# ErlerPhilipp/points2surf

Measured on NVIDIA H100. Metric: SDF queries/sec at grid_res=256, higher is better.
Workload: dtype f16 operands / f32 accumulate (wgmma); hi/lo split f16 (fp32-level) for FC tails and guard-band recompute

## Files before the change

points2surf_b200/csrc/net_tc.cu:

```cuda
#include "model.cuh"
#include "tc_ptx.cuh"

namespace p2s {

using namespace ptx;

namespace {

constexpr int kTile = 64;
constexpr int kWG = 2;
constexpr int kThreads = 128 * kWG;
template <bool PRECISE>
struct Cfg {
    static constexpr int kChunks = PRECISE ? 2 : 4;
    static constexpr int kSplit = 8 / kChunks;
    static constexpr uint32_t kChunkBytes = PRECISE ? 65536u : 32768u;
    static constexpr uint32_t kW3Bytes = kChunks * kChunkBytes;
    static constexpr uint32_t kMidScale = PRECISE ? 2u : 1u;
    static constexpr uint32_t kMidBytes = (8192u + 8192u + 16384u) * kMidScale;
    static constexpr uint32_t kPerqBytes = PRECISE ? 16384u : 8192u;
    static constexpr uint32_t kRedBytes = 4u * kChunks * 128u * 4u;
    static constexpr uint32_t kOffMid = kW3Bytes;
    static constexpr uint32_t kWgWq = kPerqBytes;
    static constexpr uint32_t kWgBytes = kWgWq + 192 * 4;
    static constexpr uint32_t kOffWg = kOffMid + kMidBytes;
    static constexpr uint32_t kOffBias = kOffWg + kWG * kWgBytes;
    static constexpr uint32_t kSlotBytes = PRECISE ? 0u : 8u * 128u * 16u;
    static constexpr uint32_t kOffSlot = kOffBias + 320 * 4;
    static constexpr uint32_t kOffXBar = kOffSlot + kWG * kSlotBytes;
    static constexpr uint32_t kSmemBytes = kOffXBar + (PRECISE ? 0u : kWG * 16u);
};
static_assert(Cfg<false>::kSmemBytes <= 232448 && Cfg<true>::kSmemBytes <= 232448, "shared memory budget");
static_assert(Cfg<false>::kRedBytes <= Cfg<false>::kPerqBytes && Cfg<true>::kRedBytes <= Cfg<true>::kPerqBytes, "reduction scratch");

struct Seg {
    const float* ptr;
    int n;
    int tiles;
    int center;
};

struct PassParams {
    Seg seg[2];
    const float* query;
    const float* R;
    int tiles_per_query;
    int B;
    const float* W0;
    const float* b0;
    int num_mid;
    int mid_N[3];
    const uint8_t* mid_img[3];
    const float* mid_bias[3];
    int perq_layer;
    const uint8_t* perq_img;
    const uint8_t* w3_img;
    float* out;
};

__device__ __forceinline__ uint32_t pack_relu(float a, float b) {
    uint32_t r;
    asm("cvt.rn.relu.satfinite.f16x2.f32 %0, %1, %2;" : "=r"(r) : "f"(b), "f"(a));
    return r;
}
__device__ __forceinline__ void pack_relu_split(float a, float b, uint32_t& hi, uint32_t& lo) {
    hi = pack_relu(a, b);
    const float2 hf = __half22float2(*reinterpret_cast<const __half2*>(&hi));
    lo = pack_half2(fmaxf(a, 0.f) - hf.x, fmaxf(b, 0.f) - hf.y);
}
template <bool PRECISE>
__device__ __forceinline__ void pack_act(float a, float b, uint32_t& hi, uint32_t& lo) {
    if (PRECISE) pack_relu_split(a, b, hi, lo);
    else hi = pack_relu(a, b);
}

template <bool PRECISE, int R>
__device__ __forceinline__ void mid_mma(float (&d)[R], const uint32_t (&a)[4], const uint32_t (&al)[4], uint64_t w, uint64_t w_lo, uint32_t acc) {
    if (R == 32) {
        auto& d32 = reinterpret_cast<float (&)[32]>(d);
        if (PRECISE) { wgmma_rs_n64(d32, al, w, acc); wgmma_rs_n64(d32, a, w_lo, 1); wgmma_rs_n64(d32, a, w, 1); }
        else wgmma_rs_n64(d32, a, w, acc);
    } else {
        auto& d64 = reinterpret_cast<float (&)[64]>(d);
        if (PRECISE) { wgmma_rs_n128(d64, al, w, acc); wgmma_rs_n128(d64, a, w_lo, 1); wgmma_rs_n128(d64, a, w, 1); }
        else wgmma_rs_n128(d64, a, w, acc);
    }
}

template <bool PRECISE, int R, int KL>
__device__ __forceinline__ void pack_acc(const float (&d)[R], const float* bias, int q4, uint32_t (&a)[R / 8][4], uint32_t (&al)[R / 8][KL]) {
#pragma unroll
    for (int j = 0; j < R / 4; ++j) {
        const float2 bb = *reinterpret_cast<const float2*>(bias + 8 * j + 2 * q4);
        pack_act<PRECISE>(d[4 * j] + bb.x, d[4 * j + 1] + bb.y, a[j >> 1][(j & 1) * 2], al[j >> 1][PRECISE ? (j & 1) * 2 : 0]);
        pack_act<PRECISE>(d[4 * j + 2] + bb.x, d[4 * j + 3] + bb.y, a[j >> 1][(j & 1) * 2 + 1], al[j >> 1][PRECISE ? (j & 1) * 2 + 1 : 0]);
    }
}

template <int S>
__device__ __forceinline__ void max_halve(float (&m)[32], int lane) {
    const bool up = (lane & S) != 0;
#pragma unroll
    for (int i = 0; i < S; ++i) {
        const float send = up ? m[i] : m[i + S], keep = up ? m[i + S] : m[i];
        m[i] = fmaxf(keep, __shfl_xor_sync(0xffffffffu, send, S));
    }
}

template <bool PRECISE>
__global__ void __launch_bounds__(kThreads, 1) pointnet_pass_kernel(const PassParams p) {
    using C = Cfg<PRECISE>;
    constexpr int kL = PRECISE ? 4 : 1;
    extern __shared__ __align__(1024) uint8_t smem[];
    float* s_bias = reinterpret_cast<float*>(smem + C::kOffBias);
    const int tid = threadIdx.x, wg = tid >> 7, t = tid & 127, lane = tid & 31, q4 = lane & 3;
    const int r0 = (t >> 5) * 16 + (lane >> 2);
    const int part = blockIdx.x % C::kSplit;
    const int stream = blockIdx.x / C::kSplit, nstreams = gridDim.x / C::kSplit;
    const int nq = (p.B > stream) ? (p.B - stream + nstreams - 1) / nstreams : 0;
    const int tpq = p.tiles_per_query;
    uint32_t mid_off[3] = {0, 0, 0};
    {
        uint32_t o = 0;
        for (int l = 0; l < (PRECISE ? p.num_mid : 3); ++l) {
            if (!PRECISE && l >= p.num_mid) break;
            mid_off[l] = o; o += (uint32_t)p.mid_N[l] * 128u * C::kMidScale;
        }
    }

    if (nq > 0) {
        const uint4* src = reinterpret_cast<const uint4*>(p.w3_img + (size_t)part * C::kW3Bytes);
        uint4* dst = reinterpret_cast<uint4*>(smem);
        for (uint32_t i = tid; i < C::kW3Bytes / 16; i += kThreads) dst[i] = src[i];
        for (int l = 0; l < (PRECISE ? p.num_mid : 3); ++l) {
            if (!PRECISE && l >= p.num_mid) break;
            if (l == p.perq_layer) continue;
            const uint4* s = reinterpret_cast<const uint4*>(p.mid_img[l]);
            uint4* d = reinterpret_cast<uint4*>(smem + C::kOffMid + mid_off[l]);
            for (uint32_t i = tid; i < (uint32_t)p.mid_N[l] * 8u * C::kMidScale; i += kThreads) d[i] = s[i];
        }
    }
    {
        int off = 0;
        for (int l = 0; l < p.num_mid; ++l) {
            for (int i = tid; i < p.mid_N[l]; i += kThreads) s_bias[off + i] = p.mid_bias[l][i];
            off += p.mid_N[l];
        }
        for (int i = tid; i < 64; i += kThreads) s_bias[256 + i] = p.b0[i];
    }
    uint64_t* xbar = reinterpret_cast<uint64_t*>(smem + C::kOffXBar);
    if (!PRECISE && tid == 0) {
        for (int w = 0; w < kWG; ++w) {
            mbar_init(xbar + 2 * w, 1);
            mbar_arrive_expect_tx(xbar + 2 * w, C::kSlotBytes);
            mbar_init(xbar + 2 * w + 1, 128);
        }
        fence_mbar_init();
    }
    fence_proxy_async_smem();
    __syncthreads();
    if (!PRECISE) cluster_sync();

    uint8_t* wsm = smem + C::kOffWg + wg * C::kWgBytes;
    uint8_t* perq = wsm;
    float* red = reinterpret_cast<float*>(perq);
    float* wq = reinterpret_cast<float*>(wsm + C::kWgWq);
    const float* s_b0 = s_bias + 256;
    const uint32_t bar_id = 1 + (uint32_t)wg;
    auto wg_sync = [&]() { asm volatile("bar.sync %0, 128;" ::"r"(bar_id) : "memory"); };
    const uint64_t dsc_w3 = make_smem_desc(smem_u32(smem), 128, 2048);
    uint64_t dsc_mid[3], dsc_mid_lo[3];
    for (int l = 0; l < 3; ++l) {
        const bool pq = l == p.perq_layer;
        dsc_mid[l] = make_smem_desc(pq ? smem_u32(perq) : smem_u32(smem + C::kOffMid) + mid_off[l], 128, 1024);
        dsc_mid_lo[l] = dsc_mid[l] + (uint64_t)((pq ? 8192u : (uint32_t)p.mid_N[l] * 128u) >> 4);
    }
    uint8_t* slot = smem + C::kOffSlot + wg * C::kSlotBytes;
    uint64_t* full = xbar + 2 * wg;
    uint64_t* empty = xbar + 2 * wg + 1;
    const uint32_t peer = (uint32_t)part ^ 1u;
    uint32_t nsend = 0, nrecv = 0;

    for (int qi = wg; qi < nq; qi += kWG) {
        const size_t q = (size_t)stream + (size_t)qi * nstreams;
        wg_sync();
        if (t < 64) {
            const float w0 = p.W0[t * 3 + 0], w1 = p.W0[t * 3 + 1], w2 = p.W0[t * 3 + 2];
            float r[9] = {1.f, 0.f, 0.f, 0.f, 1.f, 0.f, 0.f, 0.f, 1.f};
            if (p.R) {
#pragma unroll
                for (int i = 0; i < 9; ++i) r[i] = p.R[q * 9 + i];
            }
            wq[0 * 64 + t] = w0 * r[0] + w1 * r[3] + w2 * r[6];
            wq[1 * 64 + t] = w0 * r[1] + w1 * r[4] + w2 * r[7];
            wq[2 * 64 + t] = w0 * r[2] + w1 * r[5] + w2 * r[8];
        }
        if (p.perq_layer >= 0) {
            const uint4* s = reinterpret_cast<const uint4*>(p.perq_img + q * C::kPerqBytes);
            uint4* d = reinterpret_cast<uint4*>(perq);
            for (uint32_t i = t; i < C::kPerqBytes / 16; i += 128) d[i] = s[i];
            fence_proxy_async_smem();
        }
        wg_sync();
        float vmax[4 * C::kChunks];
#pragma unroll
        for (int i = 0; i < 4 * C::kChunks; ++i) vmax[i] = -INFINITY;
        const int own = PRECISE ? 0 : (part ^ wg ^ (qi >> 1)) & 1;
        for (int i = 0; i < tpq; ++i) {
            const int tq = PRECISE ? i : (i & ~1) + own;
            const bool mine = PRECISE || (!(i & 1) && tq < tpq);
            uint32_t a2[8][4], a2l[8][kL];
            if (mine) {
                const int sgi = tq < p.seg[0].tiles ? 0 : 1;
                const Seg& sg = p.seg[sgi];
                float cx = 0.f, cy = 0.f, cz = 0.f;
                if (sg.center) { cx = p.query[q * 3 + 0]; cy = p.query[q * 3 + 1]; cz = p.query[q * 3 + 2]; }
                float px[2], py[2], pz[2];
#pragma unroll
                for (int h = 0; h < 2; ++h) {
                    int local = (tq - (sgi ? p.seg[0].tiles : 0)) * kTile + r0 + 8 * h;
                    if (local >= sg.n) local = 0;
                    const float* src = sg.ptr + (q * sg.n + local) * 3;
                    px[h] = src[0] - cx; py[h] = src[1] - cy; pz[h] = src[2] - cz;
                }
                uint32_t a[4][4], al[4][kL];
#pragma unroll
                for (int kk = 0; kk < 4; ++kk) {
#pragma unroll
                    for (int hc = 0; hc < 2; ++hc) {
                        const int ch = kk * 16 + hc * 8 + 2 * q4;
                        const float2 wx = *reinterpret_cast<const float2*>(wq + 0 * 64 + ch);
                        const float2 wy = *reinterpret_cast<const float2*>(wq + 1 * 64 + ch);
                        const float2 wz = *reinterpret_cast<const float2*>(wq + 2 * 64 + ch);
                        const float2 bb = *reinterpret_cast<const float2*>(s_b0 + ch);
#pragma unroll
                        for (int h = 0; h < 2; ++h) {
                            const float v0 = fmaf(wx.x, px[h], fmaf(wy.x, py[h], fmaf(wz.x, pz[h], bb.x)));
                            const float v1 = fmaf(wx.y, px[h], fmaf(wy.y, py[h], fmaf(wz.y, pz[h], bb.y)));
                            pack_act<PRECISE>(v0, v1, a[kk][hc * 2 + h], al[kk][PRECISE ? hc * 2 + h : 0]);
                        }
                    }
                }
                const float* bl = s_bias;
#pragma unroll
                for (int l = 0; l < 2; ++l) {
                    if (l >= p.num_mid - 1) break;
                    float d[32];
#pragma unroll
                    for (int i = 0; i < 32; ++i) d[i] = 0.f;
                    wgmma_fence();
#pragma unroll
                    for (int ks = 0; ks < 4; ++ks)
                        mid_mma<PRECISE>(d, a[ks], reinterpret_cast<const uint32_t (&)[4]>(al[PRECISE ? ks : 0]), dsc_mid[l] + (uint64_t)(ks * 16), dsc_mid_lo[l] + (uint64_t)(ks * 16), ks > 0);
                    wgmma_commit();
                    wgmma_wait<0>();
                    fence_regs(d);
                    pack_acc<PRECISE>(d, bl, q4, a, al);
                    bl += 64;
                }
                {
                    const uint64_t w = p.num_mid == 3 ? dsc_mid[2] : dsc_mid[0], w_lo = p.num_mid == 3 ? dsc_mid_lo[2] : dsc_mid_lo[0];
                    float d[64];
#pragma unroll
                    for (int i = 0; i < 64; ++i) d[i] = 0.f;
                    wgmma_fence();
#pragma unroll
                    for (int ks = 0; ks < 4; ++ks)
                        mid_mma<PRECISE>(d, a[ks], reinterpret_cast<const uint32_t (&)[4]>(al[PRECISE ? ks : 0]), w + (uint64_t)(ks * 16), w_lo + (uint64_t)(ks * 16), ks > 0);
                    wgmma_commit();
                    wgmma_wait<0>();
                    fence_regs(d);
                    pack_acc<PRECISE>(d, bl, q4, a2, a2l);
                }
                if (!PRECISE) {
                    if (nsend > 0) mbar_wait_cluster_bounded(empty, (nsend - 1) & 1);
                    const uint32_t dst = mapa(smem_u32(slot), peer) + 16u * (uint32_t)t, bar = mapa(smem_u32(full), peer);
#pragma unroll
                    for (int k = 0; k < 8; ++k) st_async_v4(dst + 2048u * k, a2[k], bar);
                    ++nsend;
                }
            } else {
                mbar_wait_cluster_bounded(full, nrecv & 1);
#pragma unroll
                for (int k = 0; k < 8; ++k) {
                    const uint4 v = reinterpret_cast<const uint4*>(slot)[128 * k + t];
                    a2[k][0] = v.x; a2[k][1] = v.y; a2[k][2] = v.z; a2[k][3] = v.w;
                }
                mbar_arrive_cluster(mapa(smem_u32(empty), peer));
                if (t == 0) mbar_arrive_expect_tx(full, C::kSlotBytes);
                ++nrecv;
            }
#pragma unroll(PRECISE ? 1 : C::kChunks)
            for (int c = 0; c < C::kChunks; ++c) {
                float d[64];
#pragma unroll
                for (int i = 0; i < 64; ++i) d[i] = 0.f;
                const uint64_t w = dsc_w3 + (uint64_t)((uint32_t)c * (C::kChunkBytes >> 4));
                wgmma_fence();
#pragma unroll
                for (int ks = 0; ks < 8; ++ks) {
                    const uint64_t o = w + (uint64_t)(ks * 16);
                    if (PRECISE) {
                        wgmma_rs_n128(d, a2[ks], o + (uint64_t)(32768u >> 4), ks > 0);
                        wgmma_rs_n128(d, reinterpret_cast<const uint32_t (&)[4]>(a2l[PRECISE ? ks : 0]), o, 1);
                        wgmma_rs_n128(d, a2[ks], o, 1);
                    } else {
                        wgmma_rs_n128(d, a2[ks], o, ks > 0);
                    }
                }
                wgmma_commit();
                wgmma_wait<0>();
                fence_regs(d);
                float m[32];
#pragma unroll
                for (int j = 0; j < 16; ++j) {
                    m[2 * j] = fmaxf(d[4 * j], d[4 * j + 2]);
                    m[2 * j + 1] = fmaxf(d[4 * j + 1], d[4 * j + 3]);
                }
                max_halve<16>(m, lane);
                max_halve<8>(m, lane);
                max_halve<4>(m, lane);
                float v[4];
#pragma unroll
                for (int i = 0; i < 4; ++i) v[i] = fmaxf(vmax[i], m[i]);
#pragma unroll
                for (int i = 0; i < 4 * (C::kChunks - 1); ++i) vmax[i] = vmax[i + 4];
#pragma unroll
                for (int i = 0; i < 4; ++i) vmax[4 * (C::kChunks - 1) + i] = v[i];
            }
        }
        constexpr int kC = C::kChunks * 128;
        const int warp = t >> 5;
        wg_sync();
#pragma unroll
        for (int c = 0; c < C::kChunks; ++c)
#pragma unroll
            for (int h = 0; h < 2; ++h)
                *reinterpret_cast<float2*>(red + warp * kC + c * 128 + 16 * (lane >> 2) + 8 * h + 2 * q4) = make_float2(vmax[4 * c + 2 * h], vmax[4 * c + 2 * h + 1]);
        wg_sync();
        for (int i = t; i < kC / 4; i += 128) {
            const float4* r4 = reinterpret_cast<const float4*>(red);
            float4 v = r4[i];
#pragma unroll
            for (int w = 1; w < 4; ++w) {
                const float4 u = r4[w * (kC / 4) + i];
                v = make_float4(fmaxf(v.x, u.x), fmaxf(v.y, u.y), fmaxf(v.z, u.z), fmaxf(v.w, u.w));
            }
            *reinterpret_cast<float4*>(p.out + q * 1024 + (size_t)(part * kC + 4 * i)) = v;
        }
    }
    if (!PRECISE) cluster_sync();
}

__global__ void pack_kmajor_kernel(const float* __restrict__ W, int rows, int K, int row0, uint32_t sbo, uint8_t* __restrict__ img, int lo) {
    int e = blockIdx.x * blockDim.x + threadIdx.x;
    if (e >= rows * K) return;
    int r = e / K, k = e % K;
    uint32_t off = (uint32_t)(r >> 3) * sbo + (uint32_t)(k >> 3) * 128u + (uint32_t)(r & 7) * 16u + (uint32_t)(k & 7) * 2u;
    const float w = W[(size_t)(row0 + r) * K + k];
    const __half h = __float2half_rn(w);
    *reinterpret_cast<__half*>(img + off) = lo ? __float2half_rn(w - __half2float(h)) : h;
}

__global__ void pack_perq_kernel(const float* __restrict__ W, int64_t B, uint8_t* __restrict__ img) {
    int64_t e = (int64_t)blockIdx.x * blockDim.x + threadIdx.x;
    if (e >= B * 4096) return;
    int64_t b = e >> 12;
    int r = (int)((e >> 6) & 63), k = (int)(e & 63);
    uint32_t off = (uint32_t)(r >> 3) * 1024u + (uint32_t)(k >> 3) * 128u + (uint32_t)(r & 7) * 16u + (uint32_t)(k & 7) * 2u;
    *reinterpret_cast<__half*>(img + b * 8192 + off) = __float2half_rn(W[e]);
}

__global__ void __launch_bounds__(256) fold_w1_kernel(const float* __restrict__ W1, const float* __restrict__ T, int64_t B, uint8_t* __restrict__ img) {
    __shared__ float sW[64][65];
    __shared__ __align__(16) float sT[64][68];
    const int64_t b = blockIdx.x;
    const int tid = threadIdx.x;
    for (int e = tid; e < 4096; e += 256) {
        const int r = e >> 6, c = e & 63;
        sW[r][c] = W1[e];
        sT[r][c] = T[b * 4096 + e] + (r == c ? 1.0f : 0.0f);
    }
    __syncthreads();
    const int o = tid >> 2, i0 = (tid & 3) * 16;
    float acc[16];
#pragma unroll
    for (int i = 0; i < 16; ++i) acc[i] = 0.f;
    for (int j = 0; j < 64; ++j) {
        const float w = sW[o][j];
#pragma unroll
        for (int i4 = 0; i4 < 4; ++i4) {
            const float4 t4 = *reinterpret_cast<const float4*>(&sT[j][i0 + 4 * i4]);
            acc[4 * i4 + 0] = fmaf(w, t4.x, acc[4 * i4 + 0]);
            acc[4 * i4 + 1] = fmaf(w, t4.y, acc[4 * i4 + 1]);
            acc[4 * i4 + 2] = fmaf(w, t4.z, acc[4 * i4 + 2]);
            acc[4 * i4 + 3] = fmaf(w, t4.w, acc[4 * i4 + 3]);
        }
    }
    uint8_t* dst = img + b * 8192 + (uint32_t)(o >> 3) * 1024u + (uint32_t)(o & 7) * 16u;
#pragma unroll
    for (int h = 0; h < 2; ++h) {
        uint32_t v[4];
#pragma unroll
        for (int e = 0; e < 4; ++e) v[e] = pack_half2(acc[h * 8 + 2 * e], acc[h * 8 + 2 * e + 1]);
        *reinterpret_cast<uint4*>(dst + (uint32_t)(i0 / 8 + h) * 128u) = make_uint4(v[0], v[1], v[2], v[3]);
    }
}

__global__ void fold_fc3_kernel(const float* __restrict__ W1, const float* __restrict__ Wfc3, const float* __restrict__ bfc3,
                                float* __restrict__ G, float* __restrict__ g0) {
    const int oi = blockIdx.x;
    const int o = oi >> 6, i = oi & 63;
    const int k = threadIdx.x;
    float acc = 0.f;
    for (int j = 0; j < 64; ++j) acc = fmaf(W1[o * 64 + j], Wfc3[(size_t)(j * 64 + i) * 256 + k], acc);
    G[(size_t)oi * 256 + k] = acc;
    if (k == 0) {
        float b = W1[o * 64 + i];
        for (int j = 0; j < 64; ++j) b = fmaf(W1[o * 64 + j], bfc3[j * 64 + i], b);
        g0[oi] = b;
    }
}

__global__ void transpose64_kernel(const float* __restrict__ in, float* __restrict__ out, int64_t B) {
    int64_t e = (int64_t)blockIdx.x * blockDim.x + threadIdx.x;
    if (e >= B * 4096) return;
    int64_t b = e >> 12;
    int i = (int)((e >> 6) & 63), j = (int)(e & 63);
    out[e] = in[b * 4096 + j * 64 + i];
}

__global__ void guard_flag_kernel(const float* __restrict__ logits, int od, int64_t B, float band, int32_t* __restrict__ list, int* __restrict__ count, int64_t base, int64_t cap) {
    int64_t i = (int64_t)blockIdx.x * blockDim.x + threadIdx.x;
    if (i >= B) return;
    if (fabsf(logits[i * od + od - 1]) < band) {
        int slot = atomicAdd(count, 1);
        if (slot < cap) list[slot] = (int32_t)(base + i);
    }
}
__global__ void guard_gather_kernel(const float* __restrict__ src, const int32_t* __restrict__ list, int n, int row_floats, float* __restrict__ dst) {
    int64_t e = (int64_t)blockIdx.x * blockDim.x + threadIdx.x;
    if (e >= (int64_t)n * row_floats) return;
    int i = (int)(e / row_floats), j = (int)(e % row_floats);
    dst[e] = src[(int64_t)list[i] * row_floats + j];
}
__global__ void guard_scatter_kernel(const float* __restrict__ src, const int32_t* __restrict__ list, int n, int od, float* __restrict__ logits) {
    int i = blockIdx.x * blockDim.x + threadIdx.x;
    if (i >= n) return;
    for (int j = 0; j < od; ++j) logits[(int64_t)list[i] * od + j] = src[i * od + j];
}
__global__ void guard_scatter_rows_kernel(const float* __restrict__ src, const int32_t* __restrict__ list, int n, int row_floats, float* __restrict__ dst) {
    int64_t e = (int64_t)blockIdx.x * blockDim.x + threadIdx.x;
    if (e >= (int64_t)n * row_floats) return;
    int i = (int)(e / row_floats), j = (int)(e % row_floats);
    dst[(int64_t)list[i] * row_floats + j] = src[e];
}

}

struct TcStack {
    uint8_t* w3_img = nullptr;
    uint8_t* mid_img[3] = {nullptr, nullptr, nullptr};
    uint8_t* w3_img_p = nullptr;
    uint8_t* mid_img_p[3] = {nullptr, nullptr, nullptr};
    const float* mid_bias[3] = {nullptr, nullptr, nullptr};
    int mid_N[3] = {0, 0, 0};
    int num_mid = 0;
    const float* W0 = nullptr;
    const float* b0 = nullptr;
    const float* b3 = nullptr;
};

struct TcFc {
    const Layer* L = nullptr;
    const uint8_t* img = nullptr;
};
struct TcStnFc { TcFc fc1, fc2, fc3; };

struct TcWeights {
    TcStack qstn;
    TcStack stn[2], fin[2];
    TcStnFc qstn_fc, stn_fc[2];
    TcFc head_fc1[2], head_fc2, head_fc3;
    const uint8_t* fold_img[2] = {nullptr, nullptr};
    const float* fold_bias[2] = {nullptr, nullptr};
    TcStack stn_enc, fin_enc;
    TcStnFc stn_fc_enc;
    TcFc head_fc1_enc;
    const uint8_t* fold_img_enc = nullptr;
    const float* fold_bias_enc = nullptr;
    bool fc_on_tc = true;
    std::vector<void*> allocs;
    int sm_count = 132;
    int pass_clusters = 66;
    bool prof_on = false;
    std::vector<std::pair<cudaEvent_t, cudaEvent_t>> prof_events;
    double prof_flops = 0.0;
    ~TcWeights() {
        for (void* a : allocs) cudaFree(a);
        for (auto& e : prof_events) { cudaEventDestroy(e.first); cudaEventDestroy(e.second); }
    }
};

// ... 256 lines not shown
        launch_fc_tc_img(imgA, f.fc1.img, f.fc1.L->b, imgB, 0, Bc, 512, 1024, true, st, 3, 16, 0);
        if (out_f2) launch_fc_tc_img(imgB, f.fc2.img, f.fc2.L->b, out_f2, 256, Bc, 256, 512, true, st, 0);
        else launch_fc_tc_img(imgB, f.fc2.img, f.fc2.L->b, imgC, 0, Bc, 256, 512, true, st, 3, 8, 0);
    };
    auto qstn_rot = [&](const Layer& c3, int64_t Bc) {
        { StageScope ts("net: fc tails", st);
          if (fc_tc && img_ok(t.qstn_fc)) {
              stn_tail_img(c3, t.qstn_fc, gmax, Bc, f2);
              run_fc(t.qstn_fc.fc3, f2, 256, q4, 4, Bc, false, false, st);
          } else fc_tail(c3, t.qstn_fc, fc_tc, gmax, Bc, g, f1, f2, q4, st); }
        launch_quat_to_rot(q4, R, Bc, st);
    };
    auto stn64_perq = [&](const Feat& f, const TcStnFc& fc, const uint8_t* fold_img, const float* fold_bias, int64_t Bc) {
        if (fc_tc) {
            StageScope ts("net: fc tails", st);
            if (img_ok(fc)) {
                stn_tail_img(f.stn2.c3, fc, gmax, Bc, nullptr);
                launch_fc_tc_img(imgC, fold_img, fold_bias, perq, 0, Bc, 4096, 256, false, st, precise ? 2 : 1);
            } else {
                run_fc(fc.fc1, gmax, 1024, f1, 512, Bc, true, true, st, f.stn2.c3.b, true);
                run_fc(fc.fc2, f1, 512, f2, 256, Bc, true, true, st);
                launch_fc_tc(f2, 256, fold_img, fold_bias, reinterpret_cast<float*>(perq), 0, Bc, 4096, 256, false, st, precise ? 2 : 1);
            }
        } else {
            { StageScope ts("net: fc tails", st); fc_tail(f.stn2.c3, fc, false, gmax, Bc, g, f1, f2, T, st); }
            { StageScope ts("net: fold W1*T", st); P2S_LAUNCH(fold_w1_kernel, (unsigned)Bc, 256, 0, st, f.conv1.W, T, Bc, perq); }
        }
    };

    for (int64_t b0 = 0; b0 < B; b0 += Bc_max) {
        const int64_t Bc = (B - b0 < Bc_max) ? (B - b0) : Bc_max;
        const float* pa = patch + b0 * P * 3;
        const float* su = sub + b0 * S * 3;
        const float* qu = query + b0 * 3;
        const float* Rq = nullptr;
        if (m.single_transformer) {
            const Seg sp = make_seg(pa, P, 0), ss = make_seg(su, S, 1);
            { StageScope ts("net: pass kernels", st); launch_pass(m, t.qstn, sp, ss, qu, nullptr, Bc, -1, nullptr, gmax, st, precise); }
            qstn_rot(m.enc.stn1.c3, Bc);
            { StageScope ts("net: pass kernels", st); launch_pass(m, t.stn_enc, sp, ss, qu, R, Bc, -1, nullptr, gmax, st, precise); }
            stn64_perq(m.enc, t.stn_fc_enc, t.fold_img_enc, t.fold_bias_enc, Bc);
            { StageScope ts("net: pass kernels", st); launch_pass(m, t.fin_enc, sp, ss, qu, R, Bc, 1, perq, fmax_l, st, precise); }
            const bool fuse_b3 = fc_tc && !m.debug_aux && t.head_fc1_enc.img;
            if (!fuse_b3) launch_bias_act(fmax_l, m.enc.conv3.b, Bc, 1024, false, st);
            debug_aux_copy(m, b0, Bc, R, fmax_l, nullptr, st);
            StageScope ts_head("net: fc tails", st);
            if (fuse_b3 && t.head_fc2.img && t.head_fc3.img) {
                uint8_t* imgCat = reinterpret_cast<uint8_t*>(cat);
                launch_pack_a(fmax_l, 1024, Bc, 1024, m.enc.conv3.b, false, imgA, st);
                launch_fc_tc_img(imgA, t.head_fc1_enc.img, m.fc1_enc.b, imgCat, 0, Bc, 1024, 1024, true, st, 3, 32, 0);
                launch_fc_tc_img(imgCat, t.head_fc2.img, m.fc2.b, imgC, 0, Bc, 256, 1024, true, st, 3, 8, 0);
                launch_fc_tc_img(imgC, t.head_fc3.img, m.fc3.b, h4, 128, Bc, 128, 256, true, st, 0);
            } else {
                run_fc(t.head_fc1_enc, fmax_l, 1024, cat, 1024, Bc, true, fc_tc, st, fuse_b3 ? m.enc.conv3.b : nullptr, false);
                run_fc(t.head_fc2, cat, 1024, h3, 256, Bc, true, fc_tc, st);
                run_fc(t.head_fc3, h3, 256, h4, 128, Bc, true, fc_tc, st);
            }
            const int od = m.fc4.cout;
            launch_gemm_nt(h4, 0, 128, m.fc4.W, 0, m.fc4.b, logits + b0 * od, 0, od, (int)Bc, od, 128, 1, false, st);
            continue;
        }
        if (m.shared_qstn) {
            { StageScope ts("net: pass kernels", st); launch_pass(m, t.qstn, make_seg(pa, P, 0), make_seg(su, S, 1), qu, nullptr, Bc, -1, nullptr, gmax, st, precise); }
            qstn_rot(m.point_stn.c3, Bc);
            Rq = R;
        } else if (m.global.has_qstn) {
            launch_pass(m, t.qstn, make_seg(su, S, 1), make_seg(nullptr, 0, 0), qu, nullptr, Bc, -1, nullptr, gmax, st, precise);
            qstn_rot(m.global.stn1.c3, Bc);
            Rq = R;
        }
        for (int br = 1; br >= 0; --br) {
            const Feat& f = br ? m.global : m.local;
            const Seg sg = br ? make_seg(su, S, 1) : make_seg(pa, P, 0);
            float* fmax = br ? fmax_g : fmax_l;
            { StageScope ts("net: pass kernels", st); launch_pass(m, t.stn[br], sg, make_seg(nullptr, 0, 0), qu, Rq, Bc, -1, nullptr, gmax, st, precise); }
            stn64_perq(f, t.stn_fc[br], t.fold_img[br], t.fold_bias[br], Bc);
            (void)Tt;
            { StageScope ts("net: pass kernels", st); launch_pass(m, t.fin[br], sg, make_seg(nullptr, 0, 0), qu, Rq, Bc, 1, perq, fmax, st, precise); }
        }
        const bool fuse_b3 = fc_tc && !m.debug_aux && t.head_fc1[0].img && t.head_fc1[1].img;
        if (!fuse_b3) {
            launch_bias_act(fmax_l, m.local.conv3.b, Bc, 1024, false, st);
            launch_bias_act(fmax_g, m.global.conv3.b, Bc, 1024, false, st);
        }
        debug_aux_copy(m, b0, Bc, Rq, fmax_l, fmax_g, st);
        StageScope ts_head("net: fc tails", st);
        if (fuse_b3 && t.head_fc2.img && t.head_fc3.img) {
            uint8_t* imgCat = reinterpret_cast<uint8_t*>(cat);
            launch_pack_a(fmax_l, 1024, Bc, 1024, m.local.conv3.b, false, imgA, st);
            launch_fc_tc_img(imgA, t.head_fc1[0].img, m.fc1_local.b, imgCat, 0, Bc, 512, 1024, true, st, 3, 32, 0);
            launch_pack_a(fmax_g, 1024, Bc, 1024, m.global.conv3.b, false, imgA, st);
            launch_fc_tc_img(imgA, t.head_fc1[1].img, m.fc1_global.b, imgCat, 0, Bc, 512, 1024, true, st, 3, 32, 16);
            launch_fc_tc_img(imgCat, t.head_fc2.img, m.fc2.b, imgC, 0, Bc, 256, 1024, true, st, 3, 8, 0);
            launch_fc_tc_img(imgC, t.head_fc3.img, m.fc3.b, h4, 128, Bc, 128, 256, true, st, 0);
        } else {
            run_fc(t.head_fc1[0], fmax_l, 1024, cat, 1024, Bc, true, fc_tc, st, fuse_b3 ? m.local.conv3.b : nullptr, false);
            run_fc(t.head_fc1[1], fmax_g, 1024, cat + 512, 1024, Bc, true, fc_tc, st, fuse_b3 ? m.global.conv3.b : nullptr, false);
            run_fc(t.head_fc2, cat, 1024, h3, 256, Bc, true, fc_tc, st);
            run_fc(t.head_fc3, h3, 256, h4, 128, Bc, true, fc_tc, st);
        }
        const int od = m.fc4.cout;
        launch_gemm_nt(h4, 0, 128, m.fc4.W, 0, m.fc4.b, logits + b0 * od, 0, od, (int)Bc, od, 128, 1, false, st);
    }
}

void forward_guard(Model& m, const float* patch, const float* sub, const float* query, int64_t B, float* logits, cudaStream_t st) {
    static const bool use_fp32 = env_flag("P2S_GUARD_FP32");
    if (use_fp32) forward_fp32(m, patch, sub, query, B, logits, st);
    else forward_tc_core(m, patch, sub, query, B, logits, st, true);
}

void forward_tc(Model& m, const float* patch, const float* sub, const float* query, int64_t B,
                float* logits, cudaStream_t st) {
    const int P = m.cfg.points_per_patch, S = m.cfg.sub_sample_size, od = m.fc4.cout;
    forward_tc_core(m, patch, sub, query, B, logits, st, false);

    if (m.guard_band > 0.f && m.guard_list) {
        P2S_LAUNCH(guard_flag_kernel, (unsigned)cdiv(B, 256), 256, 0, st, logits, od, B, m.guard_band, m.guard_list, m.guard_list_count, m.guard_base, m.guard_list_cap);
    } else if (m.guard_band > 0.f) {
        StageScope ts_guard("net: guard-band fp32 recompute", st);
        int32_t* list = m.ws_guard.as<int32_t>((size_t)B + 64);
        int* count = reinterpret_cast<int*>(list + B);
        P2S_CUDA(cudaMemsetAsync(count, 0, sizeof(int), st));
        P2S_LAUNCH(guard_flag_kernel, (unsigned)cdiv(B, 256), 256, 0, st, logits, od, B, m.guard_band, list, count, (int64_t)0, B);
        int n = 0;
        P2S_CUDA(cudaMemcpyAsync(&n, count, sizeof(int), cudaMemcpyDeviceToHost, st));
        P2S_CUDA(cudaStreamSynchronize(st));
        m.last_guard_count += n;
        if (n > 0) {
            const size_t rowp = (size_t)P * 3, rows = (size_t)S * 3;
            float* const aux = m.debug_aux;
            const size_t aux_floats = aux ? (size_t)n * kAuxStride : 0;
            float* gbuf = m.ws_misc.as<float>((size_t)n * (rowp + rows + 3 + od) + 64 + aux_floats);
            float* gp = gbuf; float* gs = gp + (size_t)n * rowp; float* gq = gs + (size_t)n * rows; float* gl = gq + ((size_t)n * 3 + 3) / 4 * 4;
            float* gaux = gl + ((size_t)n * od + 3) / 4 * 4;
            P2S_LAUNCH(guard_gather_kernel, (unsigned)cdiv((int64_t)n * rowp, 256), 256, 0, st, patch, list, n, (int)rowp, gp);
            P2S_LAUNCH(guard_gather_kernel, (unsigned)cdiv((int64_t)n * rows, 256), 256, 0, st, sub, list, n, (int)rows, gs);
            P2S_LAUNCH(guard_gather_kernel, (unsigned)cdiv((int64_t)n * 3, 256), 256, 0, st, query, list, n, 3, gq);
            if (aux) m.debug_aux = gaux;
            try {
                forward_guard(m, gp, gs, gq, n, gl, st);
            } catch (...) {
                m.debug_aux = aux;
                throw;
            }
            m.debug_aux = aux;
            P2S_LAUNCH(guard_scatter_kernel, (unsigned)cdiv(n, 256), 256, 0, st, gl, list, n, od, logits);
            if (aux) P2S_LAUNCH(guard_scatter_rows_kernel, (unsigned)cdiv((int64_t)n * kAuxStride, 256), 256, 0, st, gaux, list, n, (int)kAuxStride, aux);
        }
    }
}

}
```

points2surf_b200/csrc/tc_ptx.cuh:

```cuda
#pragma once
#include <cstdint>
#include <cuda_fp16.h>

namespace p2s {
namespace ptx {

__device__ __forceinline__ uint32_t smem_u32(const void* p) { return (uint32_t)__cvta_generic_to_shared(p); }

__device__ __forceinline__ void mbar_init(uint64_t* bar, uint32_t count) {
    asm volatile("mbarrier.init.shared::cta.b64 [%0], %1;" ::"r"(smem_u32(bar)), "r"(count) : "memory");
}
__device__ __forceinline__ void fence_mbar_init() { asm volatile("fence.mbarrier_init.release.cluster;" ::: "memory"); }
__device__ __forceinline__ void mbar_arrive(uint64_t* bar) {
    asm volatile("mbarrier.arrive.shared::cta.b64 _, [%0];" ::"r"(smem_u32(bar)) : "memory");
}
__device__ __forceinline__ void mbar_arrive_expect_tx(uint64_t* bar, uint32_t bytes) {
    asm volatile("mbarrier.arrive.expect_tx.shared::cta.b64 _, [%0], %1;" ::"r"(smem_u32(bar)), "r"(bytes) : "memory");
}
__device__ __forceinline__ bool mbar_try_wait(uint64_t* bar, uint32_t parity) {
    uint32_t ok;
    asm volatile(
        "{\n\t.reg .pred p;\n\t"
        "mbarrier.try_wait.parity.shared::cta.b64 p, [%1], %2;\n\t"
        "selp.u32 %0, 1, 0, p;\n\t}"
        : "=r"(ok) : "r"(smem_u32(bar)), "r"(parity) : "memory");
    return ok != 0;
}
__device__ __forceinline__ void mbar_wait_bounded(uint64_t* bar, uint32_t parity) {
    long long t0 = clock64();
    while (!mbar_try_wait(bar, parity)) {
        if (clock64() - t0 > 2000000000LL) __trap();
    }
}
__device__ __forceinline__ bool mbar_test_wait(uint64_t* bar, uint32_t parity) {
    uint32_t ok;
    asm volatile(
        "{\n\t.reg .pred p;\n\t"
        "mbarrier.test_wait.parity.shared::cta.b64 p, [%1], %2;\n\t"
        "selp.u32 %0, 1, 0, p;\n\t}"
        : "=r"(ok) : "r"(smem_u32(bar)), "r"(parity) : "memory");
    return ok != 0;
}
__device__ __forceinline__ void mbar_wait(uint64_t* bar, uint32_t parity) {
    while (!mbar_try_wait(bar, parity)) {}
}

__device__ __forceinline__ uint32_t mapa(uint32_t addr, uint32_t rank) {
    uint32_t r;
    asm("mapa.shared::cluster.u32 %0, %1, %2;" : "=r"(r) : "r"(addr), "r"(rank));
    return r;
}
__device__ __forceinline__ void cluster_sync() {
    asm volatile("barrier.cluster.arrive.release;\n\tbarrier.cluster.wait.acquire;" ::: "memory");
}
__device__ __forceinline__ void st_async_v4(uint32_t addr, const uint32_t (&v)[4], uint32_t bar_addr) {
    asm volatile("st.async.shared::cluster.mbarrier::complete_tx::bytes.v4.b32 [%0], {%1, %2, %3, %4}, [%5];"
                 ::"r"(addr), "r"(v[0]), "r"(v[1]), "r"(v[2]), "r"(v[3]), "r"(bar_addr) : "memory");
}
__device__ __forceinline__ void mbar_arrive_cluster(uint32_t bar_addr) {
    asm volatile("mbarrier.arrive.release.cluster.shared::cluster.b64 _, [%0];" ::"r"(bar_addr) : "memory");
}
__device__ __forceinline__ bool mbar_try_wait_cluster(uint64_t* bar, uint32_t parity) {
    uint32_t ok;
    asm volatile(
        "{\n\t.reg .pred p;\n\t"
        "mbarrier.try_wait.parity.acquire.cluster.shared::cta.b64 p, [%1], %2;\n\t"
        "selp.u32 %0, 1, 0, p;\n\t}"
        : "=r"(ok) : "r"(smem_u32(bar)), "r"(parity) : "memory");
    return ok != 0;
}
__device__ __forceinline__ void mbar_wait_cluster_bounded(uint64_t* bar, uint32_t parity) {
    long long t0 = clock64();
    while (!mbar_try_wait_cluster(bar, parity)) {
        if (clock64() - t0 > 2000000000LL) __trap();
    }
}

__device__ __forceinline__ bool elect_one() {
    uint32_t pred;
    asm volatile("{\n\t.reg .pred P1;\n\telect.sync _|P1, 0xffffffff;\n\tselp.u32 %0, 1, 0, P1;\n\t}" : "=r"(pred));
    return pred != 0;
}

__device__ __forceinline__ void fence_proxy_async_smem() { asm volatile("fence.proxy.async.shared::cta;" ::: "memory"); }

__device__ __forceinline__ void bulk_g2s(void* smem_dst, const void* gmem_src, uint32_t bytes, uint64_t* bar) {
    asm volatile("cp.async.bulk.shared::cluster.global.mbarrier::complete_tx::bytes [%0], [%1], %2, [%3];"
                 ::"r"(smem_u32(smem_dst)), "l"(gmem_src), "r"(bytes), "r"(smem_u32(bar)) : "memory");
}

__device__ __forceinline__ uint64_t make_smem_desc(uint32_t smem_addr, uint32_t lbo_bytes, uint32_t sbo_bytes) {
    uint64_t d = 0;
    d |= (uint64_t)((smem_addr & 0x3FFFFu) >> 4);
    d |= (uint64_t)((lbo_bytes >> 4) & 0x3FFFu) << 16;
    d |= (uint64_t)((sbo_bytes >> 4) & 0x3FFFu) << 32;
    return d;
}

__device__ __forceinline__ void wgmma_fence() { asm volatile("wgmma.fence.sync.aligned;" ::: "memory"); }
__device__ __forceinline__ void wgmma_commit() { asm volatile("wgmma.commit_group.sync.aligned;" ::: "memory"); }
template <int N>
__device__ __forceinline__ void wgmma_wait() { asm volatile("wgmma.wait_group.sync.aligned %0;" ::"n"(N) : "memory"); }
template <int R>
__device__ __forceinline__ void fence_regs(float (&d)[R]) {
#pragma unroll
    for (int i = 0; i < R; ++i) asm volatile("" : "+f"(d[i])::"memory");
}
__device__ __forceinline__ void wgmma_rs_n64(float (&d)[32], const uint32_t (&a)[4], uint64_t b_desc, uint32_t accumulate) {
    asm volatile(
        "{\n\t.reg .pred p;\n\tsetp.ne.b32 p, %37, 0;\n\t"
        "wgmma.mma_async.sync.aligned.m64n64k16.f32.f16.f16 {%0, %1, %2, %3, %4, %5, %6, %7, %8, %9, %10, %11, %12, %13, %14, %15, %16, %17, %18, %19, %20, %21, %22, %23, %24, %25, %26, %27, %28, %29, %30, %31}, {%32, %33, %34, %35}, %36, p, 1, 1, 0;\n\t}"
        : "+f"(d[0]), "+f"(d[1]), "+f"(d[2]), "+f"(d[3]), "+f"(d[4]), "+f"(d[5]), "+f"(d[6]), "+f"(d[7]), "+f"(d[8]), "+f"(d[9]), "+f"(d[10]), "+f"(d[11]), "+f"(d[12]), "+f"(d[13]), "+f"(d[14]), "+f"(d[15]), "+f"(d[16]), "+f"(d[17]), "+f"(d[18]), "+f"(d[19]), "+f"(d[20]), "+f"(d[21]), "+f"(d[22]), "+f"(d[23]), "+f"(d[24]), "+f"(d[25]), "+f"(d[26]), "+f"(d[27]), "+f"(d[28]), "+f"(d[29]), "+f"(d[30]), "+f"(d[31])
        : "r"(a[0]), "r"(a[1]), "r"(a[2]), "r"(a[3]), "l"(b_desc), "r"(accumulate) : "memory");
}
__device__ __forceinline__ void wgmma_rs_n128(float (&d)[64], const uint32_t (&a)[4], uint64_t b_desc, uint32_t accumulate) {
    asm volatile(
        "{\n\t.reg .pred p;\n\tsetp.ne.b32 p, %69, 0;\n\t"
        "wgmma.mma_async.sync.aligned.m64n128k16.f32.f16.f16 {%0, %1, %2, %3, %4, %5, %6, %7, %8, %9, %10, %11, %12, %13, %14, %15, %16, %17, %18, %19, %20, %21, %22, %23, %24, %25, %26, %27, %28, %29, %30, %31, %32, %33, %34, %35, %36, %37, %38, %39, %40, %41, %42, %43, %44, %45, %46, %47, %48, %49, %50, %51, %52, %53, %54, %55, %56, %57, %58, %59, %60, %61, %62, %63}, {%64, %65, %66, %67}, %68, p, 1, 1, 0;\n\t}"
        : "+f"(d[0]), "+f"(d[1]), "+f"(d[2]), "+f"(d[3]), "+f"(d[4]), "+f"(d[5]), "+f"(d[6]), "+f"(d[7]), "+f"(d[8]), "+f"(d[9]), "+f"(d[10]), "+f"(d[11]), "+f"(d[12]), "+f"(d[13]), "+f"(d[14]), "+f"(d[15]), "+f"(d[16]), "+f"(d[17]), "+f"(d[18]), "+f"(d[19]), "+f"(d[20]), "+f"(d[21]), "+f"(d[22]), "+f"(d[23]), "+f"(d[24]), "+f"(d[25]), "+f"(d[26]), "+f"(d[27]), "+f"(d[28]), "+f"(d[29]), "+f"(d[30]), "+f"(d[31]), "+f"(d[32]), "+f"(d[33]), "+f"(d[34]), "+f"(d[35]), "+f"(d[36]), "+f"(d[37]), "+f"(d[38]), "+f"(d[39]), "+f"(d[40]), "+f"(d[41]), "+f"(d[42]), "+f"(d[43]), "+f"(d[44]), "+f"(d[45]), "+f"(d[46]), "+f"(d[47]), "+f"(d[48]), "+f"(d[49]), "+f"(d[50]), "+f"(d[51]), "+f"(d[52]), "+f"(d[53]), "+f"(d[54]), "+f"(d[55]), "+f"(d[56]), "+f"(d[57]), "+f"(d[58]), "+f"(d[59]), "+f"(d[60]), "+f"(d[61]), "+f"(d[62]), "+f"(d[63])
        : "r"(a[0]), "r"(a[1]), "r"(a[2]), "r"(a[3]), "l"(b_desc), "r"(accumulate) : "memory");
}
__device__ __forceinline__ void wgmma_ss_n128(float (&d)[64], uint64_t a_desc, uint64_t b_desc, uint32_t accumulate) {
    asm volatile(
        "{\n\t.reg .pred p;\n\tsetp.ne.b32 p, %66, 0;\n\t"
        "wgmma.mma_async.sync.aligned.m64n128k16.f32.f16.f16 {%0, %1, %2, %3, %4, %5, %6, %7, %8, %9, %10, %11, %12, %13, %14, %15, %16, %17, %18, %19, %20, %21, %22, %23, %24, %25, %26, %27, %28, %29, %30, %31, %32, %33, %34, %35, %36, %37, %38, %39, %40, %41, %42, %43, %44, %45, %46, %47, %48, %49, %50, %51, %52, %53, %54, %55, %56, %57, %58, %59, %60, %61, %62, %63}, %64, %65, p, 1, 1, 0, 0;\n\t}"
        : "+f"(d[0]), "+f"(d[1]), "+f"(d[2]), "+f"(d[3]), "+f"(d[4]), "+f"(d[5]), "+f"(d[6]), "+f"(d[7]), "+f"(d[8]), "+f"(d[9]), "+f"(d[10]), "+f"(d[11]), "+f"(d[12]), "+f"(d[13]), "+f"(d[14]), "+f"(d[15]), "+f"(d[16]), "+f"(d[17]), "+f"(d[18]), "+f"(d[19]), "+f"(d[20]), "+f"(d[21]), "+f"(d[22]), "+f"(d[23]), "+f"(d[24]), "+f"(d[25]), "+f"(d[26]), "+f"(d[27]), "+f"(d[28]), "+f"(d[29]), "+f"(d[30]), "+f"(d[31]), "+f"(d[32]), "+f"(d[33]), "+f"(d[34]), "+f"(d[35]), "+f"(d[36]), "+f"(d[37]), "+f"(d[38]), "+f"(d[39]), "+f"(d[40]), "+f"(d[41]), "+f"(d[42]), "+f"(d[43]), "+f"(d[44]), "+f"(d[45]), "+f"(d[46]), "+f"(d[47]), "+f"(d[48]), "+f"(d[49]), "+f"(d[50]), "+f"(d[51]), "+f"(d[52]), "+f"(d[53]), "+f"(d[54]), "+f"(d[55]), "+f"(d[56]), "+f"(d[57]), "+f"(d[58]), "+f"(d[59]), "+f"(d[60]), "+f"(d[61]), "+f"(d[62]), "+f"(d[63])
        : "l"(a_desc), "l"(b_desc), "r"(accumulate) : "memory");
}

__device__ __forceinline__ uint32_t pack_half2(float lo, float hi) {
    __half2 h = __floats2half2_rn(lo, hi);
    return *reinterpret_cast<uint32_t*>(&h);
}

}
}
```

Baseline: 431,800.

## Prefetch point tiles via cp.async and double-buffer big-layer wgmma chunks

In the fast (non-precise) path, each warp prefetches the next tile's points into shared memory with cp.async, so the first layer no longer waits on global loads. The big layer's wgmma chunks are double-buffered across two accumulator sets, and the max-reduction of one chunk overlaps the next chunk's MMA. The release of the peer's empty slot moves to after the first chunk completes and is predicated on whether the tile was received. Holding two 64-float accumulator sets raises register pressure, and optional clock-based phase tracing is added behind a compile flag.

```diff
diff --git a/points2surf_b200/csrc/net_tc.cu b/points2surf_b200/csrc/net_tc.cu
--- a/points2surf_b200/csrc/net_tc.cu
+++ b/points2surf_b200/csrc/net_tc.cu
@@ -28,7 +28,9 @@
     static constexpr uint32_t kSlotBytes = PRECISE ? 0u : 8u * 128u * 16u;
     static constexpr uint32_t kOffSlot = kOffBias + 320 * 4;
     static constexpr uint32_t kOffXBar = kOffSlot + kWG * kSlotBytes;
-    static constexpr uint32_t kSmemBytes = kOffXBar + (PRECISE ? 0u : kWG * 16u);
+    static constexpr uint32_t kPtsBytes = PRECISE ? 0u : 16u * 3u * 4u;
+    static constexpr uint32_t kOffPts = kOffXBar + (PRECISE ? 0u : kWG * 16u);
+    static constexpr uint32_t kSmemBytes = kOffPts + kWG * 4u * kPtsBytes;
 };
 static_assert(Cfg<false>::kSmemBytes <= 232448 && Cfg<true>::kSmemBytes <= 232448, "shared memory budget");
 static_assert(Cfg<false>::kRedBytes <= Cfg<false>::kPerqBytes && Cfg<true>::kRedBytes <= Cfg<true>::kPerqBytes, "reduction scratch");
@@ -106,6 +108,50 @@
         m[i] = fmaxf(keep, __shfl_xor_sync(0xffffffffu, send, S));
     }
 }
+
+template <int kChunks>
+__device__ __forceinline__ void max_chunk(const float (&d)[64], float (&vmax)[4 * kChunks], int lane) {
+    float m[32];
+#pragma unroll
+    for (int j = 0; j < 16; ++j) {
+        m[2 * j] = fmaxf(d[4 * j], d[4 * j + 2]);
+        m[2 * j + 1] = fmaxf(d[4 * j + 1], d[4 * j + 3]);
+    }
+    max_halve<16>(m, lane);
+    max_halve<8>(m, lane);
+    max_halve<4>(m, lane);
+    float v[4];
+#pragma unroll
+    for (int i = 0; i < 4; ++i) v[i] = fmaxf(vmax[i], m[i]);
+#pragma unroll
+    for (int i = 0; i < 4 * (kChunks - 1); ++i) vmax[i] = vmax[i + 4];
+#pragma unroll
+    for (int i = 0; i < 4; ++i) vmax[4 * (kChunks - 1) + i] = v[i];
+}
+
+__device__ __forceinline__ void big_chunk_mma(float (&d)[64], const uint32_t (&a2)[8][4], uint64_t w) {
+#pragma unroll
+    for (int i = 0; i < 64; ++i) d[i] = 0.f;
+    wgmma_fence();
+#pragma unroll
+    for (int ks = 0; ks < 8; ++ks) wgmma_rs_n128(d, a2[ks], w + (uint64_t)(ks * 16), ks > 0);
+    wgmma_commit();
+}
+
+#ifdef P2S_PASS_TRACE
+enum { kPhQueryStart, kPhFirst, kPhMid, kPhWaitEmpty, kPhSend, kPhBigOwn, kPhWaitFull, kPhRecv, kPhBigRecv, kPhQueryEnd, kPhases };
+__device__ unsigned long long g_pass_trace[3][kPhases];
+#define PASS_TRACE(ph)                                                  \
+    do {                                                                \
+        if (!PRECISE && t == 0) {                                       \
+            const long long now_ = clock64();                           \
+            s_trace[wg][ph] += (unsigned long long)(now_ - trace_clk);  \
+            trace_clk = now_;                                           \
+        }                                                               \
+    } while (0)
+#else
+#define PASS_TRACE(ph) do {} while (0)
+#endif
 
 template <bool PRECISE>
 __global__ void __launch_bounds__(kThreads, 1) pointnet_pass_kernel(const PassParams p) {
@@ -180,6 +226,31 @@
     uint64_t* empty = xbar + 2 * wg + 1;
     const uint32_t peer = (uint32_t)part ^ 1u;
     uint32_t nsend = 0, nrecv = 0;
+    float* pts = reinterpret_cast<float*>(smem + C::kOffPts) + (wg * 4 + (t >> 5)) * 48;
+    auto fetch_pts = [&](size_t q, int tq) {
+        const int sgi = tq < p.seg[0].tiles ? 0 : 1;
+        const Seg& sg = p.seg[sgi];
+        const int row = (tq - (sgi ? p.seg[0].tiles : 0)) * kTile + (t >> 5) * 16;
+        for (int e = lane; e < 48; e += 32) {
+            int local = row + e / 3;
+            if (local >= sg.n) local = 0;
+            cp_async_4(pts + e, sg.ptr + (q * sg.n + local) * 3 + e % 3);
+        }
+        cp_async_commit();
+    };
+    auto fetch_first = [&](int qi) {
+        for (; qi < nq; qi += kWG) {
+            const int own = (part ^ wg ^ (qi >> 1)) & 1;
+            if (own < tpq) { fetch_pts((size_t)stream + (size_t)qi * nstreams, own); return; }
+        }
+    };
+    if (!PRECISE) fetch_first(wg);
+#ifdef P2S_PASS_TRACE
+    __shared__ unsigned long long s_trace[kWG][kPhases];
+    if (t == 0)
+        for (int i = 0; i < kPhases; ++i) s_trace[wg][i] = 0;
+    long long trace_clk = clock64();
+#endif
 
     for (int qi = wg; qi < nq; qi += kWG) {
         const size_t q = (size_t)stream + (size_t)qi * nstreams;
@@ -202,6 +273,7 @@
             fence_proxy_async_smem();
         }
         wg_sync();
+        PASS_TRACE(kPhQueryStart);
         float vmax[4 * C::kChunks];
 #pragma unroll
         for (int i = 0; i < 4 * C::kChunks; ++i) vmax[i] = -INFINITY;
@@ -216,12 +288,25 @@
                 float cx = 0.f, cy = 0.f, cz = 0.f;
                 if (sg.center) { cx = p.query[q * 3 + 0]; cy = p.query[q * 3 + 1]; cz = p.query[q * 3 + 2]; }
                 float px[2], py[2], pz[2];
-#pragma unroll
-                for (int h = 0; h < 2; ++h) {
-                    int local = (tq - (sgi ? p.seg[0].tiles : 0)) * kTile + r0 + 8 * h;
-                    if (local >= sg.n) local = 0;
-                    const float* src = sg.ptr + (q * sg.n + local) * 3;
-                    px[h] = src[0] - cx; py[h] = src[1] - cy; pz[h] = src[2] - cz;
+                if (PRECISE) {
+#pragma unroll
+                    for (int h = 0; h < 2; ++h) {
+                        int local = (tq - (sgi ? p.seg[0].tiles : 0)) * kTile + r0 + 8 * h;
+                        if (local >= sg.n) local = 0;
+                        const float* src = sg.ptr + (q * sg.n + local) * 3;
+                        px[h] = src[0] - cx; py[h] = src[1] - cy; pz[h] = src[2] - cz;
+                    }
+                } else {
+                    cp_async_wait_all();
+                    __syncwarp();
+#pragma unroll
+                    for (int h = 0; h < 2; ++h) {
+                        const float* src = pts + ((lane >> 2) + 8 * h) * 3;
+                        px[h] = src[0] - cx; py[h] = src[1] - cy; pz[h] = src[2] - cz;
+                    }
+                    __syncwarp();
+                    if (tq + 2 < tpq) fetch_pts(q, tq + 2);
+                    else fetch_first(qi + kWG);
                 }
                 uint32_t a[4][4], al[4][kL];
 #pragma unroll
@@ -241,6 +326,7 @@
                         }
                     }
                 }
+                PASS_TRACE(kPhFirst);
                 const float* bl = s_bias;
 #pragma unroll
                 for (int l = 0; l < 2; ++l) {
@@ -272,62 +358,66 @@
                     fence_regs(d);
                     pack_acc<PRECISE>(d, bl, q4, a2, a2l);
                 }
+                PASS_TRACE(kPhMid);
                 if (!PRECISE) {
                     if (nsend > 0) mbar_wait_cluster_bounded(empty, (nsend - 1) & 1);
+                    PASS_TRACE(kPhWaitEmpty);
                     const uint32_t dst = mapa(smem_u32(slot), peer) + 16u * (uint32_t)t, bar = mapa(smem_u32(full), peer);
 #pragma unroll
                     for (int k = 0; k < 8; ++k) st_async_v4(dst + 2048u * k, a2[k], bar);
                     ++nsend;
+                    PASS_TRACE(kPhSend);
                 }
             } else {
                 mbar_wait_cluster_bounded(full, nrecv & 1);
+                PASS_TRACE(kPhWaitFull);
 #pragma unroll
                 for (int k = 0; k < 8; ++k) {
                     const uint4 v = reinterpret_cast<const uint4*>(slot)[128 * k + t];
                     a2[k][0] = v.x; a2[k][1] = v.y; a2[k][2] = v.z; a2[k][3] = v.w;
                 }
-                mbar_arrive_cluster(mapa(smem_u32(empty), peer));
                 if (t == 0) mbar_arrive_expect_tx(full, C::kSlotBytes);
                 ++nrecv;
+                PASS_TRACE(kPhRecv);
             }
-#pragma unroll(PRECISE ? 1 : C::kChunks)
-            for (int c = 0; c < C::kChunks; ++c) {
-                float d[64];
-#pragma unroll
-                for (int i = 0; i < 64; ++i) d[i] = 0.f;
-                const uint64_t w = dsc_w3 + (uint64_t)((uint32_t)c * (C::kChunkBytes >> 4));
-                wgmma_fence();
-#pragma unroll
-                for (int ks = 0; ks < 8; ++ks) {
-                    const uint64_t o = w + (uint64_t)(ks * 16);
-                    if (PRECISE) {
+            if constexpr (PRECISE) {
+#pragma unroll 1
+                for (int c = 0; c < C::kChunks; ++c) {
+                    float d[64];
+#pragma unroll
+                    for (int i = 0; i < 64; ++i) d[i] = 0.f;
+                    const uint64_t w = dsc_w3 + (uint64_t)((uint32_t)c * (C::kChunkBytes >> 4));
+                    wgmma_fence();
+#pragma unroll
+                    for (int ks = 0; ks < 8; ++ks) {
+                        const uint64_t o = w + (uint64_t)(ks * 16);
                         wgmma_rs_n128(d, a2[ks], o + (uint64_t)(32768u >> 4), ks > 0);
-                        wgmma_rs_n128(d, reinterpret_cast<const uint32_t (&)[4]>(a2l[PRECISE ? ks : 0]), o, 1);
+                        wgmma_rs_n128(d, reinterpret_cast<const uint32_t (&)[4]>(a2l[ks]), o, 1);
                         wgmma_rs_n128(d, a2[ks], o, 1);
+                    }
+                    wgmma_commit();
+                    wgmma_wait<0>();
+                    fence_regs(d);
+                    max_chunk<C::kChunks>(d, vmax, lane);
+                }
+            } else {
+                float d[2][64];
+                big_chunk_mma(d[0], a2, dsc_w3);
+#pragma unroll
+                for (int c = 0; c < C::kChunks; ++c) {
+                    if (c + 1 < C::kChunks) {
+                        big_chunk_mma(d[(c + 1) & 1], a2, dsc_w3 + (uint64_t)((uint32_t)(c + 1) * (C::kChunkBytes >> 4)));
+                        wgmma_wait<1>();
                     } else {
-                        wgmma_rs_n128(d, a2[ks], o, ks > 0);
+                        wgmma_wait<0>();
                     }
+                    fence_regs(d[c & 1]);
+                    if (c == 0) mbar_arrive_cluster(mapa(smem_u32(empty), peer), !mine);
+                    max_chunk<C::kChunks>(d[c & 1], vmax, lane);
                 }
-                wgmma_commit();
-                wgmma_wait<0>();
-                fence_regs(d);
-                float m[32];
-#pragma unroll
-                for (int j = 0; j < 16; ++j) {
-                    m[2 * j] = fmaxf(d[4 * j], d[4 * j + 2]);
-                    m[2 * j + 1] = fmaxf(d[4 * j + 1], d[4 * j + 3]);
-                }
-                max_halve<16>(m, lane);
-                max_halve<8>(m, lane);
-                max_halve<4>(m, lane);
-                float v[4];
-#pragma unroll
-                for (int i = 0; i < 4; ++i) v[i] = fmaxf(vmax[i], m[i]);
-#pragma unroll
-                for (int i = 0; i < 4 * (C::kChunks - 1); ++i) vmax[i] = vmax[i + 4];
-#pragma unroll
-                for (int i = 0; i < 4; ++i) vmax[4 * (C::kChunks - 1) + i] = v[i];
             }
+            if (mine) PASS_TRACE(kPhBigOwn);
+            else PASS_TRACE(kPhBigRecv);
         }
         constexpr int kC = C::kChunks * 128;
         const int warp = t >> 5;
@@ -348,7 +438,14 @@
             }
             *reinterpret_cast<float4*>(p.out + q * 1024 + (size_t)(part * kC + 4 * i)) = v;
         }
-    }
+        PASS_TRACE(kPhQueryEnd);
+    }
+#ifdef P2S_PASS_TRACE
+    if (!PRECISE && t == 0) {
+        const int cls = p.num_mid == 1 ? 0 : (p.seg[0].center ? 2 : 1);
+        for (int i = 0; i < kPhases; ++i) atomicAdd(&g_pass_trace[cls][i], s_trace[wg][i]);
+    }
+#endif
     if (!PRECISE) cluster_sync();
 }
 
@@ -911,3 +1008,13 @@
 }
 
 }
+
+#ifdef P2S_PASS_TRACE
+extern "C" int p2s_pass_trace_read(unsigned long long* out, int reset) {
+    if (cudaDeviceSynchronize() != cudaSuccess) return 1;
+    if (cudaMemcpyFromSymbol(out, p2s::g_pass_trace, sizeof(p2s::g_pass_trace)) != cudaSuccess) return 1;
+    static const unsigned long long zero[3][p2s::kPhases] = {};
+    if (reset && cudaMemcpyToSymbol(p2s::g_pass_trace, zero, sizeof(zero)) != cudaSuccess) return 1;
+    return 0;
+}
+#endif
diff --git a/points2surf_b200/csrc/tc_ptx.cuh b/points2surf_b200/csrc/tc_ptx.cuh
--- a/points2surf_b200/csrc/tc_ptx.cuh
+++ b/points2surf_b200/csrc/tc_ptx.cuh
@@ -57,8 +57,9 @@
     asm volatile("st.async.shared::cluster.mbarrier::complete_tx::bytes.v4.b32 [%0], {%1, %2, %3, %4}, [%5];"
                  ::"r"(addr), "r"(v[0]), "r"(v[1]), "r"(v[2]), "r"(v[3]), "r"(bar_addr) : "memory");
 }
-__device__ __forceinline__ void mbar_arrive_cluster(uint32_t bar_addr) {
-    asm volatile("mbarrier.arrive.release.cluster.shared::cluster.b64 _, [%0];" ::"r"(bar_addr) : "memory");
+__device__ __forceinline__ void mbar_arrive_cluster(uint32_t bar_addr, bool arrive) {
+    asm volatile("{\n\t.reg .pred p;\n\tsetp.ne.b32 p, %1, 0;\n\t@p mbarrier.arrive.shared::cluster.b64 _, [%0];\n\t}"
+                 ::"r"(bar_addr), "r"((uint32_t)arrive) : "memory");
 }
 __device__ __forceinline__ bool mbar_try_wait_cluster(uint64_t* bar, uint32_t parity) {
     uint32_t ok;
@@ -88,6 +89,12 @@
     asm volatile("cp.async.bulk.shared::cluster.global.mbarrier::complete_tx::bytes [%0], [%1], %2, [%3];"
                  ::"r"(smem_u32(smem_dst)), "l"(gmem_src), "r"(bytes), "r"(smem_u32(bar)) : "memory");
 }
+
+__device__ __forceinline__ void cp_async_4(void* smem_dst, const void* gmem_src) {
+    asm volatile("cp.async.ca.shared.global [%0], [%1], 4;" ::"r"(smem_u32(smem_dst)), "l"(gmem_src) : "memory");
+}
+__device__ __forceinline__ void cp_async_commit() { asm volatile("cp.async.commit_group;" ::: "memory"); }
+__device__ __forceinline__ void cp_async_wait_all() { asm volatile("cp.async.wait_group 0;" ::: "memory"); }
 
 __device__ __forceinline__ uint64_t make_smem_desc(uint32_t smem_addr, uint32_t lbo_bytes, uint32_t sbo_bytes) {
     uint64_t d = 0;
```

Result: faster. 464,200 (median of 6 runs) (+7.5%).
